# arkworks-rs/accumulation

Hardware: AMD Instinct MI355X
Metric: MSM throughput (point-scalar pairs/sec) at 2^20 Pallas (higher is better)
Workload: dtype u32; 1 GPU; 2^20-pair pallas MSM per GPU (north_star size; scalars uniform in [0, r), G_i = k_i*G), key resident + precomputed window multiples; pairs_per_gpu=1048576, curve=pallas, precomputed_key=True, parallelism=point-sharded x1, window_bits=20, pipeline=bucket-per-lane (k_prep_local_t + k_accum_bpl; skewed scalars re-run chunked), window_widths=9 x 20 + 4 x 19 bits = 256 (MsmGeom::n_narrow), msms_in_flight=3, full=False

## Files before the change

accumulation_amd/csrc/api_entry_ctx.inc:

```

const char* amsm_strerror(int s) {
  switch (s) {
    case AMSM_OK: return "ok";
    case AMSM_E_INVALID_ARG: return "invalid argument";
    case AMSM_E_OOM: return "out of (device) memory";
    case AMSM_E_HIP: return "HIP runtime error";
    case AMSM_E_UNSUPPORTED: return "unsupported size or configuration";
    case AMSM_E_NO_DEVICE: return "no usable gfx950 device (the host backend is never chosen implicitly: ask for AMSM_DEVICE_HOST)";
    case AMSM_E_SCALAR_RANGE: return "scalar out of range (not a canonical into_repr value)";
    case AMSM_E_RCCL: return "RCCL collective failed";
    case AMSM_E_INVALID_POINT: return "invalid point (non-canonical, off the curve or outside the prime-order subgroup)";
    default: return "unknown error";
  }
}

int amsm_device_count(void) {
  int n = 0;
  if (hipGetDeviceCount(&n) != hipSuccess) {
    (void)hipGetLastError();
    return 0;
  }
  return n;
}

// ... 63 lines not shown
    if (hipGetDeviceProperties(&prop, device_id) == hipSuccess && prop.multiProcessorCount > 0) {
      c->cu_count = prop.multiProcessorCount;
      int per_cu = with_curve(curve, [](auto cv) { return accum_l0_blocks_per_cu<typename decltype(cv)::Fq>(); });
      c->wave_slots = prop.multiProcessorCount * std::max(1, per_cu) * 4;
    }
  }
  c->pool_cap_bytes = pool_cap_from_env(c->pool_cap_bytes);
  c->gate.limit = mem_limit_from_env();
  if (const char* e = getenv("AMSM_BPL")) c->bpl = atoi(e) != 0;
  if (const char* e = getenv("AMSM_BPL_PLAIN")) c->bpl_plain = atoi(e) != 0;
  if (const char* e = getenv("AMSM_TOP_SETS")) {
    const int t = atoi(e);
    c->top_sets = (t == 2 || t == 4 || t == 8) ? t : 0;
  }
  if (const char* e = getenv("AMSM_BPL_PROBE")) c->bpl_probe = atoi(e) != 0;
  if (const char* e = getenv("AMSM_BPS")) c->bps = std::max(0, std::min(2, atoi(e)));
  if (const char* e = getenv("AMSM_BPS_BATCH")) c->bps_batch = std::max(0, std::min((int)msel::BPS_BATCH, atoi(e)));
  if (const char* e = getenv("AMSM_SPLIT_LOG2")) c->split_log2 = std::max(0, std::min(28, atoi(e)));
  if (const char* e = getenv("AMSM_DIRECT_SUM_MAX_LOG2")) c->direct_max_log2 = std::max(0, std::min(16, atoi(e)));
  if (const char* e = getenv("AMSM_TWO_VALUED")) c->two_valued = atoi(e) != 0;
  if (const char* e = getenv("AMSM_SHARE_BUCKETS")) c->share_buckets = atoi(e) != 0;
  if (const char* e = getenv("AMSM_HOST_HALVES")) c->host_halves = atoi(e) != 0;
  if (const char* e = getenv("AMSM_SUBGROUP_LADDER")) c->subgroup_ladder = atoi(e) == 2 ? 2 : 1;
  if (const char* e = getenv("AMSM_VEC_SAMPLE_FORM")) c->vec_sample_form = std::max(0, std::min(2, atoi(e)));
  *out = c;
  return AMSM_OK;
}

void amsm_ctx_destroy(amsm_ctx* c) {
  if (!c) return;
// ... 280 lines not shown
```

accumulation_amd/csrc/api_pipeline.inc:

```

#define HIP_TRY(expr)                                                                                  \
  do {                                                                                                 \
    hipError_t _e = (expr);                                                                            \
    if (_e != hipSuccess) {                                                                            \
      fprintf(stderr, "[amsm] HIP error %s (%d) at %s:%d: %s\n", hipGetErrorName(_e), (int)_e, __FILE__, \
              __LINE__, #expr);                                                                        \
      return _e == hipErrorOutOfMemory ? AMSM_E_OOM : AMSM_E_HIP;                                      \
    }                                                                                                  \
  } while (0)

#define TRY(expr)            \
  do {                       \
    int _s = (expr);         \
    if (_s != AMSM_OK) return _s; \
  } while (0)

int ensure(DevBuf& b, size_t bytes) {
  if (b.bytes >= bytes && b.p) return AMSM_OK;
  if (b.p) HIP_TRY(gate_free(b.p));
  b.p = nullptr;
  b.bytes = 0;
  size_t want = bytes + bytes / 8 + 256;
  TRY(gate_alloc(b.owner, GATE_DEVICE, want, false, &b.p));
  b.bytes = want;
// ... 335 lines not shown
  const size_t rec = xyzz_bytes<Fq>();
  if (direct_sum_applies(ctx, job)) {
    DirectPlan dp;
    if (eff) *eff = bases;
    *short_prep_out = false;
    return direct_plan<Fq>(ctx, sl, &job, 1, &dp);
  }
  const msel::Choice ch = choose_pipeline(ctx, bases, n, group_shift, job.force_chunked);
  auto common = [&]() -> int {
    TRY(ensure(sl->buckets, (size_t)g.B * rec));
    return reserve_tail<Fq>(ctx, sl, g.n_sets, msel::tail_plan_any_place(g.nb, g.n_sets, g.B, g.E, g.bpl == 1u));
  };
  if (ch.pipeline == msel::BUCKET_PER_LANE && bpl_geom(ctx, bases, base_off, n, group_shift, ch.plain_window, &g)) {
    sl->geom = g;
    if (eff) *eff = bases;
    TRY(ensure(sl->vals_a, prep_bpl_part_entries(g) * 8 + 64));
    TRY(ensure(sl->vals_b, (size_t)prep_bpl_partitions(g) * prep_bpl_stride(g) * 4 + 64));
    TRY(ensure(sl->bpl_grp, (size_t)prep_bpl_partitions(g) * prep_bpl_groups_per_partition() * 8 + 64));
    TRY(ensure(sl->bpl_order, (size_t)prep_bpl_partitions(g) * prep_bpl_groups_per_partition() * 64 * 4 + 64));
    TRY(common());
    TRY(ensure(sl->prep_small, 64 + prep_small_words(g) * sizeof(u32) + 256));
    *short_prep_out = true;
    return AMSM_OK;
  }
  if (bases->bpl) TRY(bases_alt<Fq>(ctx, bases, &bases));
  if (eff) *eff = bases;
  if (ch.pipeline == msel::BUCKET_SPLIT && bps_geom(ctx, bases, base_off, n, group_shift, &g)) {
    sl->geom = g;
    const u32 P = prep_bps_partitions(g, g.bps_log2_l);
    TRY(ensure(sl->vals_a, prep_bps_part_entries(g, g.bps_log2_l) * 4 + 64));
    TRY(ensure(sl->vals_b, (size_t)P * prep_bps_stride(g, g.bps_log2_l) * 4 + 64));
// ... 107 lines not shown
  u32* d_heavy_count = d_err + 1;
  u32* vals_a = (u32*)sl->vals_a.p;
  u32* vals_b = (u32*)sl->vals_b.p;

  auto prep = [&]() -> int {
    if (!short_prep) HIP_TRY(hipMemsetAsync(sl->misc.p, 0, 64, st));
    stage_mark(ctx, sl, ST_DIGITS, st);
    if (g.bpl) {
      PrepBplBuffers pb;
      pb.d_small = d_err + 16;
      pb.part = vals_a;
      pb.ents_t = vals_b;
      pb.grp = sl->bpl_grp.p;
      pb.order = (u32*)sl->bpl_order.p;
      pb.err = d_err;
      const int rc = g.bpl == 2 ? launch_prep_bps<Fr>(st, (const u32*)d_scalars, scalars_mont, g, g.bps_log2_l, pb)
                                : launch_prep_bpl<Fr>(st, (const u32*)d_scalars, scalars_mont, g, pb);
      if (rc != 0) return AMSM_E_HIP;
      stage_mark(ctx, sl, ST_SORT, st);
      stage_mark(ctx, sl, ST_BOUNDS, st);
      if (g.bpl != 2) ctx->n_bpl++;
      else if (!job.counted) ctx->n_bps++;
      if (g.bpl == 1u && g.top_split) ctx->n_top_sets[(g.top_split + 1u) / 4u]++;
    } else if (short_prep) {
      PrepBuffers pb;
      pb.d_small = d_err + 16;
      pb.part = vals_a;
      pb.vals_sorted = vals_b;
      pb.start = (u32*)sl->start.p;
      pb.items = (u32*)sl->items.p;
// ... 1117 lines not shown
```

accumulation_amd/csrc/api_types.h:

```cpp
#pragma once
struct amsm_ctx;
namespace {

enum Stage { ST_DIGITS = 0, ST_SORT, ST_BOUNDS, ST_ACCUM_L0, ST_ACCUM_L12, ST_REDUCE, ST_COUNT };
const char* kStageNames[ST_COUNT] = {"prep_chain", "prep_sort_rocprim", "prep_bounds_rocprim", "accum_l0", "accum_l1_l2",
                                     "bucket_reduce_fold"};

struct DevBuf {
  void* p = nullptr;
  size_t bytes = 0;
  amsm_ctx* owner = nullptr;
  void release();
};

struct MemGate {
  size_t held = 0, peak = 0;
  size_t limit = 0;
  size_t pinned = 0;
  unsigned long long requests = 0, refused_limit = 0, refused_hook = 0, failed_driver = 0;
  long fail_after = -1;
};

}

// ... 156 lines not shown
  int cu_count = 256;
  unsigned vec_grid_max = 0;
  int wave_slots = 4096;
  bool bpl = true;
  bool bpl_plain = true;
  int top_sets = 0;
  int bps = 2;
  int split_log2 = 21;
  unsigned long long n_bps = 0, n_bps_fallbacks = 0;
  int bps_batch = msel::BPS_BATCH;
  unsigned long long n_bps_units = 0, n_bps_batched = 0, n_bps_unit_reruns = 0;
  unsigned long long n_direct = 0;
  int direct_max_log2 = 15;
  unsigned direct_rr = 0;
  bool host_halves = true;
  bool bpl_probe = true;
  unsigned long long n_top_sets[3] = {0, 0, 0};
  unsigned long long n_bpl = 0, n_bpl_fallbacks = 0;
  bool share_buckets = true;
  DevBuf shared_buckets[2];
  hipEvent_t shared_free[2] = {};
  bool shared_used[2] = {false, false};
  unsigned shared_rr = 0;
  unsigned long long n_shared = 0;
  size_t table_budget = ~(size_t)0;
  unsigned long long n_tables_denied = 0;
  bool profiling = false;
  float stage_ms[ST_COUNT] = {};
  float stage_acc[ST_COUNT] = {};
  int stage_n = 0;
// ... 111 lines not shown
```

accumulation_amd/csrc/kern_fr.hip:

```cpp
#include "launch.h"
#include "vec_kernels.h"
#include "prep_kernels.h"

#include <algorithm>
#include <cmath>
#include <atomic>
#include <cstdlib>
#include <cstring>

namespace amsm {

static inline u32 cdiv_(u32 a, u32 b) { return (a + b - 1) / b; }
void launch_bounds(hipStream_t st, const void* keys_sorted, bool keys16, u32* vals_sorted, MsmGeom g, u32* start,
                   u32* items) {
  if (keys16)
    hipLaunchKernelGGL((k_bounds<uint16_t>), dim3(cdiv_(g.B, 256)), dim3(256), 0, st, (const uint16_t*)keys_sorted,
                       vals_sorted, g, start, items);
  else
    hipLaunchKernelGGL((k_bounds<u32>), dim3(cdiv_(g.B, 256)), dim3(256), 0, st, (const u32*)keys_sorted, vals_sorted,
                       g, start, items);
}

constexpr u32 PREP_MAX_P = 4096;
static PrepGeom prep_geom(const MsmGeom& g) {
// ... 53 lines not shown
  unsigned long long max_idx = (unsigned long long)g.base_off + g.n - 1ull +
                               (g.precomp ? (unsigned long long)(g.W - 1u) * g.table_stride : 0ull);
  if (g.idx_rel_bits) max_idx = ((unsigned long long)(g.W - 1u) << g.idx_rel_bits) | ((1ull << g.idx_rel_bits) - 1ull);
  pg.IB = 1;
  while ((max_idx >> pg.IB) != 0ull) pg.IB++;
  pg.CAP = BPL_LOCAL_BUDGET_WORDS - BPL_LOCAL_FIXED_WORDS;
  pg.HEAVY = 0xffffffffu;
  const unsigned long long per = std::max<unsigned long long>(((unsigned long long)g.E + pg.P - 1) / std::max(1u, pg.P), g.part_max);
  pg.FIX = (u32)std::min<unsigned long long>(pg.CAP, (per + per / 4ull + 2048ull + 15ull) & ~15ull);
  return pg;
}
size_t prep_bpl_part_entries(const MsmGeom& g) {
  PrepGeom pg = prep_bpl_geom(g);
  return std::max<size_t>(g.E, pg.FIX ? (size_t)pg.P * pg.FIX : 0);
}
static size_t prep_bpl_local_lds(const PrepGeom& pg) { return (size_t)(BPL_LOCAL_FIXED_WORDS + pg.CAP) * sizeof(u32); }
static size_t prep_bpl_scatter_lds(const MsmGeom& g, const PrepGeom& pg) {
  const size_t cap = (size_t)pg.SPB * g.S;
  return (3 * (size_t)pg.P + 2 * cap) * sizeof(u32) + cap * sizeof(uint16_t);
}
u32 prep_bpl_partitions(const MsmGeom& g) { return g.B >> 10; }
u32 prep_bpl_groups_per_partition() { return BPL_GROUPS; }
u32 prep_bpl_stride(const MsmGeom& g) {
  const u32 P = std::max(1u, prep_bpl_partitions(g));
  const unsigned long long per = std::max<unsigned long long>(((unsigned long long)g.E + P - 1) / P, g.part_max);
  return (u32)((per + per / 4ull + 4096ull + 1023ull) & ~1023ull);
}
bool prep_bpl_supported(const MsmGeom& g) {
  if (g.S > 32u || g.n == 0 || g.n_sets != g.groups * sets_per_group(g)) return false;
  if (g.B < (1u << 16) || (g.B & 1023u) || (g.B >> 10) > PREP_MAX_P || ((g.B >> 10) & 3u)) return false;
  PrepGeom pg = prep_bpl_geom(g);
  if (pg.IB > 30u) return false;
  if (!msel::bpl_stage_fits(g.E, pg.P, g.part_max, pg.CAP)) return false;
  return prep_bpl_scatter_lds(g, pg) <= PREP_LDS_LIMIT && prep_bpl_local_lds(pg) <= PREP_LDS_LIMIT &&
         (unsigned long long)pg.P * prep_bpl_stride(g) < (1ull << 31);
}
static std::atomic<unsigned long long> prep_bpl_attr_devices{0};
template <class KS>
static void prep_bpl_attr(KS scatter_kernel) {
  int dev = 0;
  if (hipGetDevice(&dev) != hipSuccess || dev < 0 || dev >= 64) dev = 63;
  const unsigned long long bit = 1ull << dev;
  (void)hipFuncSetAttribute((const void*)scatter_kernel, hipFuncAttributeMaxDynamicSharedMemorySize, (int)PREP_LDS_LIMIT);
  if (dev != 63 && (prep_bpl_attr_devices.load(std::memory_order_acquire) & bit)) return;
  static_assert((BPL_LOCAL_BUDGET_WORDS) * sizeof(u32) <= PREP_LDS_LIMIT, "k_prep_local_t's LDS must fit a workgroup");
  (void)hipFuncSetAttribute((const void*)k_prep_local_t, hipFuncAttributeMaxDynamicSharedMemorySize, (int)PREP_LDS_LIMIT);
  prep_bpl_attr_devices.fetch_or(bit, std::memory_order_release);
}

constexpr u32 bps_local_fixed_words(u32 nbp) { return 4u * nbp + 1024u + BPL_BINS + 2u * BPS_GROUPS + 2u; }
constexpr u32 BPS_LOCAL_BUDGET_WORDS = 37888u;
static PrepGeom prep_bps_geom(const MsmGeom& g, u32 log2_l) {
  PrepGeom pg;
  pg.SH = 10u - log2_l;
  pg.P = g.B >> pg.SH;
  pg.SPB = g.S <= 16u ? 512u : 256u;
  unsigned long long max_idx = (unsigned long long)g.base_off + g.n - 1ull +
                               (g.precomp ? (unsigned long long)(g.W - 1u) * g.table_stride : 0ull);
  if (g.idx_rel_bits) max_idx = ((unsigned long long)(g.W - 1u) << g.idx_rel_bits) | ((1ull << g.idx_rel_bits) - 1ull);
  pg.IB = 1;
  while ((max_idx >> pg.IB) != 0ull) pg.IB++;
// ... 208 lines not shown
    PrepGeom pg = prep_bpl_geom(g);                                                                                  \
    u32* part_total = b.d_small;                                                                                     \
    u32* part_start = b.d_small + (PREP_MAX_P + 1);                                                                  \
    u32* part_cursor = b.d_small + 2 * (PREP_MAX_P + 1);                                                             \
    PrepHeavy hv;                                                                                                    \
    hv.n = b.d_small + 4 * (PREP_MAX_P + 1);                                                                         \
    hv.cnt = hv.n + 1;                                                                                               \
    hv.ids = hv.cnt + 64;                                  \
    hv.cur = hv.end = hv.ids;                                                                                        \
    {                  \
      size_t zero_bytes = (16 + 4 * (PREP_MAX_P + 1) + 1) * sizeof(u32);                                             \
      zero_bytes = (zero_bytes + 255) & ~(size_t)255;                                                                \
      if (b.err != b.d_small - 16) return -1;                                                                        \
      if (hipMemsetAsync(b.err, 0, zero_bytes, st) != hipSuccess) return -1;                                         \
    }                                                                                                                \
    if (g.S <= 16u) prep_bpl_attr(k_prep_scatter<FR, 16, 1, true>);                                                  \
    else prep_bpl_attr(k_prep_scatter<FR, 32, 1, true>);                                                             \
    if (!pg.FIX) {                                                                                                   \
      PrepGeom ph = pg;                                                                                              \
      ph.SPB = 1024;                                                                                                 \
      hipLaunchKernelGGL((k_prep_hist<FR>), dim3(cdiv_(g.n, 1024)), dim3(1024), pg.P * sizeof(u32), st, scalars,      \
                         mont, g, ph, part_total, b.err);                                                            \
      hipLaunchKernelGGL(k_prep_scan, dim3(1), dim3(1024), 0, st, part_total, part_start, pg.P, pg.HEAVY, hv);       \
    }                                                                                                                \
    if (g.S <= 16u)                                                                                                  \
      hipLaunchKernelGGL((k_prep_scatter<FR, 16, 1, true>), dim3(cdiv_(g.n, pg.SPB)), dim3(512),                     \
                         prep_bpl_scatter_lds(g, pg), st, scalars, mont, g, pg, part_start, part_cursor, b.part, b.err); \
    else                                             \
      hipLaunchKernelGGL((k_prep_scatter<FR, 32, 1, true>), dim3(cdiv_(g.n, pg.SPB)), dim3(256),                     \
                         prep_bpl_scatter_lds(g, pg), st, scalars, mont, g, pg, part_start, part_cursor, b.part, b.err); \
    hipLaunchKernelGGL(k_prep_local_t, dim3(pg.P), dim3(1024), prep_bpl_local_lds(pg), st,                           \
                       pg.FIX ? part_cursor : part_start, (const u64*)b.part, g, pg, prep_bpl_stride(g), b.ents_t,   \
                       (BplGroup*)b.grp, b.order, b.err);                                                            \
    return 0;                                                                                                        \
  }                                                                                                                  \
  template <>                                                                                                        \
  void launch_digits<FR>(hipStream_t st, const u32* scalars, int mont, MsmGeom g, void* keys, bool keys16, u32* vals, \
                         u32* err) {                                                                                 \
    if (keys16)                                                                                                      \
      hipLaunchKernelGGL((k_digits<FR, uint16_t>), dim3(cdiv_(g.n, 256)), dim3(256), 0, st, scalars, mont, g,         \
                         (uint16_t*)keys, vals, err);                                                                \
    else                                                                                                             \
      hipLaunchKernelGGL((k_digits<FR, u32>), dim3(cdiv_(g.n, 256)), dim3(256), 0, st, scalars, mont, g, (u32*)keys,  \
                         vals, err);                                                                                 \
  }                                                                                                                  \
  template <>                                                                                                        \
  void launch_skew_probe<FR>(hipStream_t st, const u32* scalars, int mont, u32 n, DigitWalk walk, u32* d_flag,       \
                             const u32* d_tv_words) {                                                               \
// ... 125 lines not shown
```

accumulation_amd/csrc/launch.h:

```cpp
#pragma once
#include <hip/hip_runtime.h>

#include <algorithm>

#include "blind.h"
#include "msm_select.h"
#include "msm_types.h"

namespace amsm {

template <class Fq>
void launch_accum_l0(hipStream_t st, const u32* table, const u32* vals_sorted, const u32* start,
                     const u32* item_off, MsmGeom g, u32* partials);
template <class Fq>
void launch_accum_bpl(hipStream_t st, const u32* table, const u32* ents_t, const void* grp, const u32* order, u32 n_groups,
                      u32 groups_per_part, const u32* flags, u32* buckets, u32 wg_per_cu = 0, bool accumulate = false);
template <class Fq>
int accum_l0_blocks_per_cu();
template <class Fq>
void launch_accum_l1(hipStream_t st, u32 lanes_per_bucket, const u32* partials, const u32* items, const u32* item_off, MsmGeom g,
                     u32* buckets, u32* heavy_count, u32* heavy_list);
template <class Fq>
void launch_accum_l2(hipStream_t st, const u32* partials, const u32* items, const u32* item_off,
                     const u32* heavy_count, const u32* heavy_list, u32* scratch, u32* buckets);
// ... 63 lines not shown
  u32* part;
  u32* vals_sorted;
  u32* start;
  u32* items;
  u32* item_off;
  u32* err;
};
bool prep_supported(const MsmGeom& g);
struct PrepBplBuffers {
  u32* d_small;
  u32* part;
  u32* ents_t;
  void* grp;
  u32* order;
  u32* err;
};
bool prep_bpl_supported(const MsmGeom& g);
u32 prep_bpl_stride(const MsmGeom& g);
u32 prep_bpl_partitions(const MsmGeom& g);
size_t prep_bpl_part_entries(const MsmGeom& g);
size_t prep_bps_part_entries(const MsmGeom& g, u32 log2_l);
u32 prep_bpl_groups_per_partition();
template <class Fr>
int launch_prep_bpl(hipStream_t st, const u32* scalars, int mont, MsmGeom g, const PrepBplBuffers& b);
int prep_bps_choose(const MsmGeom& g);
u32 prep_bps_partitions(const MsmGeom& g, u32 log2_l);
u32 prep_bps_stride(const MsmGeom& g, u32 log2_l);
template <class Fr>
int launch_prep_bps(hipStream_t st, const u32* scalars, int mont, MsmGeom g, u32 log2_l, const PrepBplBuffers& b);
template <class Fq>
void launch_accum_bps(hipStream_t st, const u32* table, const u32* ents_t, const void* grp, const u32* order, u32 n_groups,
                      u32 log2_l, const u32* flags, u32* buckets);
struct BpsBatchBuffers {
  u32* small;
  u32 small_stride;
// ... 76 lines not shown
```

accumulation_amd/csrc/msm_select.h:

```cpp
#pragma once
#include <math.h>
#include <stddef.h>

#include <initializer_list>

namespace amsm {
namespace msel {

enum Pipeline { DIRECT_SUM = 0, BUCKET_SPLIT = 1, BUCKET_PER_LANE = 2, CHUNKED = 3 };
inline const char* pipeline_name(int p) {
  return p == DIRECT_SUM ? "direct_sum" : (p == BUCKET_SPLIT ? "bucket_split" : (p == BUCKET_PER_LANE ? "bucket_per_lane" : "chunked"));
}

inline int ilog2_ceil(size_t n) {
  int l = 0;
  while (((size_t)1 << l) < n) l++;
  return l;
}
constexpr size_t P2(int k) { return (size_t)1 << k; }

constexpr int BPL_WINDOW = 20;
constexpr int DIRECT_MAX_LOG2 = 15;
struct KeyWindowRow {
  int lg_lo, lg_hi;
// ... 194 lines not shown
      const char *a0 = vec[v].scalars, *a1 = a0 + vec[v].n * 32;
      for (size_t u = 0; u < k && verdict[v] == V_ONES_APART; u++) {
        if (u == v || verdict[u] != V_REGULAR || vec[u].n == 0) continue;
        const char *b0 = vec[u].scalars, *b1 = b0 + vec[u].n * 32;
        if (a0 < b1 && b0 < a1) verdict[v] = V_REGULAR, changed = true;
      }
    }
  }
}

constexpr unsigned BPL_STAGE_CAP = 37340;
inline bool bpl_stage_fits(unsigned long long E, unsigned long long P, unsigned long long part_max, unsigned cap) {
  if (P == 0 || E / P + 1024ull > cap) return false;
  return !(part_max && part_max + 5ull * (unsigned long long)sqrt((double)part_max) > cap);
}
inline unsigned long long plain_part_max(size_t n, unsigned nb, unsigned long long reach, unsigned T, unsigned groups) {
  const unsigned long long per_win = ((unsigned long long)n * 1024ull + nb - 1) / nb;
  const unsigned long long per_top = ((unsigned long long)n * 1024ull + reach - 1) / reach;
  const unsigned long long top = (2ull * per_top + T - 1) / T;
  const unsigned long long pm = per_win > top ? per_win : top;
  return groups > 1u ? (pm + 1ull) / 2ull : pm;
}
inline unsigned plain_top_sets(size_t n, unsigned nb, unsigned long long reach, unsigned W, unsigned groups, unsigned cap = BPL_STAGE_CAP,
                               unsigned max_sets = 8) {
  if (n == 0 || nb < 1024u || reach == 0 || W == 0) return 0;
  for (unsigned T = 2; T <= max_sets && T <= 8u; T *= 2u) {
    const unsigned long long P = ((unsigned long long)groups * (W + T) * nb) >> 10;
    if (bpl_stage_fits((unsigned long long)n * W, P, plain_part_max(n, nb, reach, T, groups), cap)) return T;
  }
  return 0;
// ... 82 lines not shown
```

accumulation_amd/csrc/prep_kernels.h:

```cpp
#pragma once
#include "fp.h"
#include "msm_select.h"
#include "msm_types.h"
#include "vec_kernels.h"

namespace amsm {

struct PrepGeom {
  u32 SH;
  u32 P;
  u32 SPB;
  u32 IB;
  u32 CAP;
  u32 HEAVY;
  u32 FIX;
};

constexpr u32 PREP_HEAVY_SLICES = 64, PREP_HEAVY_GRID = 1024, PREP_MAX_HEAVY = 4096;
struct PrepHeavy {
  u32* n;
  u32* ids;
  u32* cnt;
  u32* cur;
  u32* end;
};

constexpr u32 PREP_ENTRY_LAST = 0x40000000u;

AMSM_DEV u32 lds_count(u32* ctr, u32 idx) {
  const u64 active = __ballot(1);
// ... 91 lines not shown
    u32 v = in[k];
    out[k] = run;
    run += v;
  }
  if (with_total && t == T - 1) out[n] = lds[T - 1];
}

__global__ void __launch_bounds__(1024)
    k_prep_scan(const u32* __restrict__ part_total, u32* __restrict__ part_start, u32 P, u32 heavy_min, PrepHeavy hv) {
  __shared__ u32 lds[1024];
  block_exclusive_scan(part_total, part_start, P, true, lds);
  for (u32 p = threadIdx.x; p < P; p += blockDim.x)
    if (part_total[p] > heavy_min) hv.ids[atomicAdd(hv.n, 1u)] = p;
}

template <class Fr, int MAXW, int SPT, bool WIDE>
AMSM_DEV void prep_scatter_body(const u32* scalars, int mont, MsmGeom g, PrepGeom pg, const u32* part_start, u32* part_cursor, u32* part,
                                u32* err) {
  extern __shared__ u32 prep_lds[];
  const u32 cap = pg.SPB * g.S;
  u32* cnt = prep_lds;
  u32* loff = prep_lds + pg.P;
  u32* gbase = prep_lds + 2 * pg.P;
  u32* staged = prep_lds + 3 * pg.P;
  uint16_t* staged_p = reinterpret_cast<uint16_t*>(staged + (WIDE ? 2u : 1u) * cap);
  const u32 t = threadIdx.x, T = blockDim.x;
  for (u32 p = t; p < pg.P; p += T) cnt[p] = 0;
  __syncthreads();
  u32 rk[SPT][MAXW / 2];
  Fe<Fr> sreg[SPT];
#pragma unroll
  for (int r = 0; r < SPT; r++) {
#pragma unroll
// ... 3 lines not shown
      sreg[r] = fe_load<Fr>(scalars + (size_t)i * 8);
      if (g.skip_ones) fe_drop_stored_one<Fr>(sreg[r], mont);
      if (mont) sreg[r] = fe_from_mont<Fr>(sreg[r]);
      const u32 bad = scalar_entries_unrolled_reg<Fr, MAXW>(sreg[r], g, i, [&](int w, u32 key, u32) {
        u32 rank = atomicAdd(&cnt[key >> pg.SH], 1u);
        rk[r][w >> 1] |= rank << ((w & 1) * 16);
      });
      if (pg.FIX && bad && err) atomicOr(err, 1u);
    }
  }
  __syncthreads();
  constexpr u32 RSV_MAX = 4;
  u32 rsv[RSV_MAX], rsv_base[RSV_MAX];
  u32 per = (pg.P + T - 1) / T;
  u32 lo = min(t * per, pg.P), hi = min(lo + per, pg.P);
  {
    u32* sl = reinterpret_cast<u32*>(staged);
    u32 sum = 0;
    for (u32 p = lo; p < hi; p++) sum += cnt[p];
    sl[t] = sum;
    __syncthreads();
    for (u32 d = 1; d < T; d <<= 1) {
      u32 v = t >= d ? sl[t - d] : 0u;
      __syncthreads();
      sl[t] += v;
      __syncthreads();
    }
    u32 run = sl[t] - sum;
#pragma unroll
    for (u32 q = 0; q < RSV_MAX; q++) {
      u32 p = lo + q;
      rsv[q] = 0;
      rsv_base[q] = 0;
      if (p < hi) {
        u32 v = cnt[p];
        loff[p] = run;
        if (v) {
          rsv_base[q] = pg.FIX ? p * pg.FIX : part_start[p];
          rsv[q] = atomicAdd(&part_cursor[p], v);
        }
        run += v;
      }
    }
    for (u32 p = lo + RSV_MAX; p < hi; p++) {
      u32 v = cnt[p];
      loff[p] = run;
      gbase[p] = v ? (pg.FIX ? p * pg.FIX : part_start[p]) + atomicAdd(&part_cursor[p], v) : 0u;
      run += v;
    }
  }
  __syncthreads();
  const u32 low = (1u << pg.SH) - 1u;
#pragma unroll
  for (int r = 0; r < SPT; r++) {
    u32 i = blockIdx.x * pg.SPB + r * T + t;
    if (i < g.n)
      scalar_entries_unrolled_reg<Fr, MAXW>(sreg[r], g, i, [&](int w, u32 key, u32 val) {
        u32 p = key >> pg.SH;
        u32 rank = (rk[r][w >> 1] >> ((w & 1) * 16)) & 0xffffu;
        u32 slot = loff[p] + rank;
        if (WIDE) reinterpret_cast<u64*>(staged)[slot] = ((u64)(key & low) << 32) | val;
        else staged[slot] = (val & 0x80000000u) | ((key & low) << pg.IB) | (val & 0x7fffffffu);
        staged_p[slot] = (uint16_t)p;
      });
  }
#pragma unroll
  for (u32 q = 0; q < RSV_MAX; q++)
    if (lo + q < hi) gbase[lo + q] = rsv_base[q] + rsv[q];
  __syncthreads();
  u32 total = loff[pg.P - 1] + cnt[pg.P - 1];
  for (u32 j = t; j < total; j += T) {
    u32 p = staged_p[j];
    const u32 dst = gbase[p] + (j - loff[p]);
    if (pg.FIX && dst - p * pg.FIX >= pg.FIX) continue;
    if (WIDE) reinterpret_cast<u64*>(part)[dst] = reinterpret_cast<const u64*>(staged)[j];
    else part[dst] = staged[j];
  }
}
template <class Fr, int MAXW, int SPT, bool WIDE = false>
__global__ void __launch_bounds__(512)
    k_prep_scatter(const u32* __restrict__ scalars, int mont, MsmGeom g, PrepGeom pg, const u32* __restrict__ part_start,
                   u32* __restrict__ part_cursor, u32* __restrict__ part, u32* __restrict__ err = nullptr) {
  prep_scatter_body<Fr, MAXW, SPT, WIDE>(scalars, mont, g, pg, part_start, part_cursor, part, err);
}
constexpr int PREP_BPS_BATCH = msel::BPS_BATCH;
struct BpsBatchScalars {
  const u32* scalars[PREP_BPS_BATCH];
};
template <class Fr, int MAXW, int SPT>
__global__ void __launch_bounds__(512)
    k_prep_scatter_batch(BpsBatchScalars b, int mont, MsmGeom g, PrepGeom pg, const u32* __restrict__ part_start0,
                         u32* __restrict__ part_cursor0, u32 small_stride, u32* __restrict__ part0, u32 part_stride,
                         u32* __restrict__ err) {
  const size_t v = blockIdx.y;
  prep_scatter_body<Fr, MAXW, SPT, false>(b.scalars[v], mont, g, pg, part_start0 + v * small_stride, part_cursor0 + v * small_stride,
                                          part0 + v * part_stride, err);
}

// ... 250 lines not shown
  __syncthreads();
  u32 before = 0;
#pragma unroll
  for (u32 i = 0; i < 15u; i++) before += i < w ? wt[i] : 0u;
  return v + before;
}

constexpr u32 BPL_LOCAL_SLOTS = 37, BPL_SLOT_BLOCK = 8;
template <class F>
AMSM_DEV void bpl_slot_blocks(u32 n, F&& f) {
#pragma unroll
  for (u32 b = 0; b < BPL_LOCAL_SLOTS; b += BPL_SLOT_BLOCK)
    if (b * BPL_NB < n) f(b);
}

__global__ void __launch_bounds__(1024)
    k_prep_local_t(const u32* __restrict__ part_start, const u64* __restrict__ part, MsmGeom g, PrepGeom pg, u32 stride,
                   u32* __restrict__ ents_t, BplGroup* __restrict__ grp, u32* __restrict__ order, u32* __restrict__ err) {
  extern __shared__ u32 prep_lds[];
  constexpr u32 NB = BPL_NB, NG = BPL_GROUPS, T = BPL_NB, SLOTS = BPL_LOCAL_SLOTS, BLK = BPL_SLOT_BLOCK;
  u32* cnt = prep_lds;
  u32* cur = cnt + NB;
  u32* wt = cur + NB;
  u32* bins = wt + NB;
  u32* first = bins + BPL_BINS;
  u32* gm = first + BPL_BINS;
  u32* stage = gm + 2u * NG + 1u;
  const u32 p = blockIdx.x, t = threadIdx.x;
  const u32 ps = pg.FIX ? p * pg.FIX : part_start[p];
  const u32 n_p = pg.FIX ? part_start[p] : part_start[p + 1] - ps;
  const u32 pe = ps + (pg.FIX ? min(n_p, pg.FIX) : n_p);
  const u32 low = NB - 1u, idx_mask = (1u << pg.IB) - 1u, b0 = p << pg.SH;
  const bool fits = n_p <= pg.CAP && (!pg.FIX || n_p <= pg.FIX);
  const u32 n = fits ? min(pe - ps, SLOTS * T) : 0u;
  u64 e[SLOTS];
#pragma unroll
  for (u32 i = 0; i < SLOTS; i++) e[i] = 0;
  bpl_slot_blocks(n, [&](u32 b) {
#pragma unroll
    for (u32 i = b; i < b + BLK && i < SLOTS; i++) e[i] = part[ps + min(i * T + t, n - 1u)];
  });
  cnt[t] = 0;
  if (t < BPL_BINS) bins[t] = 0;
  if (t < NG) gm[t] = 0;
  __syncthreads();
  bpl_slot_blocks(n, [&](u32 b) {
#pragma unroll
    for (u32 i = b; i < b + BLK && i < SLOTS; i++)
      if (i * T + t < n) atomicAdd(&cnt[(u32)(e[i] >> 32) & low], 1u);
  });
  __syncthreads();
  const u32 c_t = cnt[t];
  const u32 first_t = block_scan_inclusive(c_t, wt) - c_t;
  cur[t] = first_t;
  const u32 bin = min(c_t, BPL_BINS - 1u);
  const u32 rank = atomicAdd(&bins[bin], 1u);
  __syncthreads();
  bpl_slot_blocks(n, [&](u32 b) {
    u32 pos[BLK];
#pragma unroll
    for (u32 i = b; i < b + BLK && i < SLOTS; i++) {
      pos[i - b] = 0;
      if (i * T + t < n) pos[i - b] = atomicAdd(&cur[(u32)(e[i] >> 32) & low], 1u);
    }
#pragma unroll
    for (u32 i = b; i < b + BLK && i < SLOTS; i++) {
      const u32 lo = (u32)e[i];
      if (i * T + t < n) stage[pos[i - b]] = (lo & 0x80000000u) | entry_abs_index(g, lo & idx_mask);
    }
  });
  const u32 in_class = t < BPL_BINS ? bins[BPL_BINS - 1u - t] : 0u;
  const u32 larger = block_scan_inclusive(in_class, wt + 16) - in_class;
  if (t < BPL_BINS) first[BPL_BINS - 1u - t] = larger;
  __syncthreads();
  const u32 my_pos = first[bin] + rank;
  cnt[my_pos] = c_t;
  cur[my_pos] = first_t;
  {
    const u32 h0 = (c_t + 1u) >> 1;
    if (my_pos < BPL_SPLIT / 2u) atomicMax(&gm[0], h0);
    else if (my_pos < BPL_SPLIT) atomicMax(&gm[NG - 1u], h0);
    else atomicMax(&gm[my_pos / BPL_GROUP], c_t);
  }
  __syncthreads();
  u32 total = 0, my_gb = 0;
// ... 161 lines not shown
```

Baseline: 986.5 million pairs/s.

## Pack bucket-per-lane prep entries into one 32-bit word with sub-range cursors

Adds a narrow entry form for the bucket-per-lane prep. Each partition entry becomes one u32 holding the sign, local bucket and window, plus a point offset relative to a sub-range. Points are split into G sub-ranges with their own cursors and capacities. The aim is to halve the global traffic and the scatter LDS between k_prep_scatter and k_prep_local_t. The cost is extra geometry logic and more capacity-overflow conditions, and the wide u64 form is kept behind AMSM_BPL_WIDE as a fallback.

```diff
diff --git a/accumulation_amd/csrc/api_entry_ctx.inc b/accumulation_amd/csrc/api_entry_ctx.inc
--- a/accumulation_amd/csrc/api_entry_ctx.inc
+++ b/accumulation_amd/csrc/api_entry_ctx.inc
@@ -101,6 +101,7 @@
     c->top_sets = (t == 2 || t == 4 || t == 8) ? t : 0;
   }
   if (const char* e = getenv("AMSM_BPL_PROBE")) c->bpl_probe = atoi(e) != 0;
+  if (const char* e = getenv("AMSM_BPL_WIDE")) c->bpl_wide = atoi(e) != 0;
   if (const char* e = getenv("AMSM_BPS")) c->bps = std::max(0, std::min(2, atoi(e)));
   if (const char* e = getenv("AMSM_BPS_BATCH")) c->bps_batch = std::max(0, std::min((int)msel::BPS_BATCH, atoi(e)));
   if (const char* e = getenv("AMSM_SPLIT_LOG2")) c->split_log2 = std::max(0, std::min(28, atoi(e)));
diff --git a/accumulation_amd/csrc/api_pipeline.inc b/accumulation_amd/csrc/api_pipeline.inc
--- a/accumulation_amd/csrc/api_pipeline.inc
+++ b/accumulation_amd/csrc/api_pipeline.inc
@@ -373,7 +373,7 @@
   if (ch.pipeline == msel::BUCKET_PER_LANE && bpl_geom(ctx, bases, base_off, n, group_shift, ch.plain_window, &g)) {
     sl->geom = g;
     if (eff) *eff = bases;
-    TRY(ensure(sl->vals_a, prep_bpl_part_entries(g) * 8 + 64));
+    TRY(ensure(sl->vals_a, prep_bpl_part_entries(g) * prep_bpl_entry_bytes(g, ctx->bpl_wide) + 64));
     TRY(ensure(sl->vals_b, (size_t)prep_bpl_partitions(g) * prep_bpl_stride(g) * 4 + 64));
     TRY(ensure(sl->bpl_grp, (size_t)prep_bpl_partitions(g) * prep_bpl_groups_per_partition() * 8 + 64));
     TRY(ensure(sl->bpl_order, (size_t)prep_bpl_partitions(g) * prep_bpl_groups_per_partition() * 64 * 4 + 64));
@@ -511,6 +511,7 @@
       pb.grp = sl->bpl_grp.p;
       pb.order = (u32*)sl->bpl_order.p;
       pb.err = d_err;
+      pb.wide = ctx->bpl_wide;
       const int rc = g.bpl == 2 ? launch_prep_bps<Fr>(st, (const u32*)d_scalars, scalars_mont, g, g.bps_log2_l, pb)
                                 : launch_prep_bpl<Fr>(st, (const u32*)d_scalars, scalars_mont, g, pb);
       if (rc != 0) return AMSM_E_HIP;
diff --git a/accumulation_amd/csrc/api_types.h b/accumulation_amd/csrc/api_types.h
--- a/accumulation_amd/csrc/api_types.h
+++ b/accumulation_amd/csrc/api_types.h
@@ -194,6 +194,7 @@
   int direct_max_log2 = 15;
   unsigned direct_rr = 0;
   bool host_halves = true;
+  bool bpl_wide = false;
   bool bpl_probe = true;
   unsigned long long n_top_sets[3] = {0, 0, 0};
   unsigned long long n_bpl = 0, n_bpl_fallbacks = 0;
diff --git a/accumulation_amd/csrc/kern_fr.hip b/accumulation_amd/csrc/kern_fr.hip
--- a/accumulation_amd/csrc/kern_fr.hip
+++ b/accumulation_amd/csrc/kern_fr.hip
@@ -91,10 +91,24 @@
   PrepGeom pg = prep_bpl_geom(g);
   return std::max<size_t>(g.E, pg.FIX ? (size_t)pg.P * pg.FIX : 0);
 }
+static_assert(msel::BPL_SUB_BUCKET_BITS == 10 && BPL_NB == (1u << msel::BPL_SUB_BUCKET_BITS), "a partition is 2^10 buckets");
+static_assert(msel::BPL_SUB_MAX * msel::BPL_SUB_SLOTS * BPL_NB >= BPL_LOCAL_BUDGET_WORDS - BPL_LOCAL_FIXED_WORDS,
+              "k_prep_local_t<false>'s register slots hold a whole stage");
+static_assert(msel::BPL_SUB_MAX * msel::BPL_SUB_SLOTS <= 2u * BPL_LOCAL_SLOTS, "one-word slots take no more registers than the wide ones");
+static_assert(msel::BPL_SUB_FIX_CONST == 2048u, "prep_bpl_geom: the constant of FIX");
+constexpr u32 BPL_CURSOR_WORDS = 2u * (PREP_MAX_P + 1u);
+static msel::BplEntryForm prep_bpl_form(const MsmGeom& g, const PrepGeom& pg, bool wide) {
+  const unsigned long long per = std::max<unsigned long long>(((unsigned long long)g.E + pg.P - 1) / std::max(1u, pg.P), g.part_max);
+  const msel::BplEntryForm f = msel::bpl_entry_form(g.n, g.W, g.precomp != 0u, pg.P, per, pg.FIX, BPL_CURSOR_WORDS, wide);
+  if (f.narrow && f.G > 1u && g.groups > 1u && g.group_shift >= f.lbits)
+    return msel::bpl_entry_form(g.n, g.W, g.precomp != 0u, pg.P, per, pg.FIX, BPL_CURSOR_WORDS, true);
+  return f;
+}
+size_t prep_bpl_entry_bytes(const MsmGeom& g, bool wide) { return prep_bpl_form(g, prep_bpl_geom(g), wide).narrow ? 4 : 8; }
 static size_t prep_bpl_local_lds(const PrepGeom& pg) { return (size_t)(BPL_LOCAL_FIXED_WORDS + pg.CAP) * sizeof(u32); }
-static size_t prep_bpl_scatter_lds(const MsmGeom& g, const PrepGeom& pg) {
+static size_t prep_bpl_scatter_lds(const MsmGeom& g, const PrepGeom& pg, bool narrow = false) {
   const size_t cap = (size_t)pg.SPB * g.S;
-  return (3 * (size_t)pg.P + 2 * cap) * sizeof(u32) + cap * sizeof(uint16_t);
+  return (3 * (size_t)pg.P + (narrow ? 1 : 2) * cap) * sizeof(u32) + cap * sizeof(uint16_t);
 }
 u32 prep_bpl_partitions(const MsmGeom& g) { return g.B >> 10; }
 u32 prep_bpl_groups_per_partition() { return BPL_GROUPS; }
@@ -121,7 +135,8 @@
   (void)hipFuncSetAttribute((const void*)scatter_kernel, hipFuncAttributeMaxDynamicSharedMemorySize, (int)PREP_LDS_LIMIT);
   if (dev != 63 && (prep_bpl_attr_devices.load(std::memory_order_acquire) & bit)) return;
   static_assert((BPL_LOCAL_BUDGET_WORDS) * sizeof(u32) <= PREP_LDS_LIMIT, "k_prep_local_t's LDS must fit a workgroup");
-  (void)hipFuncSetAttribute((const void*)k_prep_local_t, hipFuncAttributeMaxDynamicSharedMemorySize, (int)PREP_LDS_LIMIT);
+  (void)hipFuncSetAttribute((const void*)k_prep_local_t<true>, hipFuncAttributeMaxDynamicSharedMemorySize, (int)PREP_LDS_LIMIT);
+  (void)hipFuncSetAttribute((const void*)k_prep_local_t<false>, hipFuncAttributeMaxDynamicSharedMemorySize, (int)PREP_LDS_LIMIT);
   prep_bpl_attr_devices.fetch_or(bit, std::memory_order_release);
 }
 
@@ -360,6 +375,28 @@
       if (b.err != b.d_small - 16) return -1;                                                                        \
       if (hipMemsetAsync(b.err, 0, zero_bytes, st) != hipSuccess) return -1;                                         \
     }                                                                                                                \
+    const msel::BplEntryForm form = prep_bpl_form(g, pg, b.wide);                                                    \
+    if (form.narrow) {           \
+      PrepSub sub;                                                                                                   \
+      sub.G = form.G;                                                                                                \
+      sub.lbits = form.lbits;                                                                                        \
+      sub.wmask = (1u << form.wbits) - 1u;                                                                           \
+      sub.stride = form.cap_full;                                                                                    \
+      sub.cap_full = form.cap_full;                                                                                  \
+      sub.cap_last = form.cap_last;                                                                                  \
+      if (g.S <= 16u) {                                                                                              \
+        prep_bpl_attr(k_prep_scatter_sub<FR, 16, 1>);                                                                \
+        hipLaunchKernelGGL((k_prep_scatter_sub<FR, 16, 1>), dim3(cdiv_(g.n, pg.SPB)), dim3(512),                     \
+                           prep_bpl_scatter_lds(g, pg, true), st, scalars, mont, g, pg, sub, part_cursor, b.part, b.err); \
+      } else {                                                                                                       \
+        prep_bpl_attr(k_prep_scatter_sub<FR, 32, 1>);                                                                \
+        hipLaunchKernelGGL((k_prep_scatter_sub<FR, 32, 1>), dim3(cdiv_(g.n, pg.SPB)), dim3(256),                     \
+                           prep_bpl_scatter_lds(g, pg, true), st, scalars, mont, g, pg, sub, part_cursor, b.part, b.err); \
+      }                                                                                                              \
+      hipLaunchKernelGGL(k_prep_local_t<false>, dim3(pg.P), dim3(1024), prep_bpl_local_lds(pg), st, part_cursor,     \
+                         (const void*)b.part, g, pg, sub, prep_bpl_stride(g), b.ents_t, (BplGroup*)b.grp, b.order, b.err); \
+      return 0;                                                                                                      \
+    }                                                                                                                \
     if (g.S <= 16u) prep_bpl_attr(k_prep_scatter<FR, 16, 1, true>);                                                  \
     else prep_bpl_attr(k_prep_scatter<FR, 32, 1, true>);                                                             \
     if (!pg.FIX) {                                                                                                   \
@@ -375,9 +412,9 @@
     else                                             \
       hipLaunchKernelGGL((k_prep_scatter<FR, 32, 1, true>), dim3(cdiv_(g.n, pg.SPB)), dim3(256),                     \
                          prep_bpl_scatter_lds(g, pg), st, scalars, mont, g, pg, part_start, part_cursor, b.part, b.err); \
-    hipLaunchKernelGGL(k_prep_local_t, dim3(pg.P), dim3(1024), prep_bpl_local_lds(pg), st,                           \
-                       pg.FIX ? part_cursor : part_start, (const u64*)b.part, g, pg, prep_bpl_stride(g), b.ents_t,   \
-                       (BplGroup*)b.grp, b.order, b.err);                                                            \
+    hipLaunchKernelGGL(k_prep_local_t<true>, dim3(pg.P), dim3(1024), prep_bpl_local_lds(pg), st,                     \
+                       pg.FIX ? part_cursor : part_start, (const void*)b.part, g, pg, PrepSub{}, prep_bpl_stride(g), \
+                       b.ents_t, (BplGroup*)b.grp, b.order, b.err);                                                  \
     return 0;                                                                                                        \
   }                                                                                                                  \
   template <>                                                                                                        \
diff --git a/accumulation_amd/csrc/launch.h b/accumulation_amd/csrc/launch.h
--- a/accumulation_amd/csrc/launch.h
+++ b/accumulation_amd/csrc/launch.h
@@ -101,11 +101,13 @@
   void* grp;
   u32* order;
   u32* err;
+  bool wide = false;
 };
 bool prep_bpl_supported(const MsmGeom& g);
 u32 prep_bpl_stride(const MsmGeom& g);
 u32 prep_bpl_partitions(const MsmGeom& g);
 size_t prep_bpl_part_entries(const MsmGeom& g);
+size_t prep_bpl_entry_bytes(const MsmGeom& g, bool wide);
 size_t prep_bps_part_entries(const MsmGeom& g, u32 log2_l);
 u32 prep_bpl_groups_per_partition();
 template <class Fr>
diff --git a/accumulation_amd/csrc/msm_select.h b/accumulation_amd/csrc/msm_select.h
--- a/accumulation_amd/csrc/msm_select.h
+++ b/accumulation_amd/csrc/msm_select.h
@@ -232,6 +232,51 @@
   if (P == 0 || E / P + 1024ull > cap) return false;
   return !(part_max && part_max + 5ull * (unsigned long long)sqrt((double)part_max) > cap);
 }
+constexpr unsigned BPL_SUB_MAX = 8, BPL_SUB_SLOTS = 5, BPL_SUB_BUCKET_BITS = 10, BPL_SUB_FIX_CONST = 2048;
+struct BplEntryForm {
+  unsigned narrow;
+  unsigned wbits;
+  unsigned lbits;
+  unsigned G;
+  unsigned cap_full;
+  unsigned cap_last;
+  unsigned slots;
+};
+inline BplEntryForm bpl_entry_form(unsigned long long n, unsigned W, bool precomp, unsigned long long P, unsigned long long per,
+                                   unsigned fix, unsigned long long cursor_words, bool force_wide) {
+  BplEntryForm f{};
+  f.G = 1;
+  f.cap_full = f.cap_last = fix;
+  if (force_wide || fix == 0 || n == 0 || P == 0) return f;
+  unsigned wbits = 0;
+  if (precomp)
+    while (((W - 1u) >> wbits) != 0u) wbits++;
+  const unsigned room = 31u - BPL_SUB_BUCKET_BITS;
+  if (wbits + 9u > room) return f;
+  const unsigned lbits = room - wbits;
+  const unsigned long long full = 1ull << lbits, G = (n + full - 1ull) / full;
+  if (G > BPL_SUB_MAX || P * G > cursor_words) return f;
+  if (G == 1ull) {
+    if (fix > BPL_SUB_MAX * BPL_SUB_SLOTS * 1024u) return f;
+    f.slots = (fix + 1023u) / 1024u;
+  } else {
+    const unsigned long long last = n - (G - 1ull) * full;
+    const unsigned long long b_full = per * full / n, b_last = per * last / n, k = BPL_SUB_FIX_CONST / G;
+    f.cap_full = (unsigned)((b_full + b_full / 4ull + k) & ~15ull);
+    f.cap_last = (unsigned)((b_last + b_last / 4ull + k) & ~15ull);
+    if (f.cap_full > BPL_SUB_SLOTS * 1024u || (G - 1ull) * f.cap_full + f.cap_last > fix) {
+      f.cap_full = f.cap_last = fix;
+      return f;
+    }
+    f.slots = (unsigned)(G - 1ull) * ((f.cap_full + 1023u) / 1024u) + (f.cap_last + 1023u) / 1024u;
+  }
+  f.narrow = 1;
+  f.wbits = wbits;
+  f.lbits = lbits;
+  f.G = (unsigned)G;
+  return f;
+}
+
 inline unsigned long long plain_part_max(size_t n, unsigned nb, unsigned long long reach, unsigned T, unsigned groups) {
   const unsigned long long per_win = ((unsigned long long)n * 1024ull + nb - 1) / nb;
   const unsigned long long per_top = ((unsigned long long)n * 1024ull + reach - 1) / reach;
diff --git a/accumulation_amd/csrc/prep_kernels.h b/accumulation_amd/csrc/prep_kernels.h
--- a/accumulation_amd/csrc/prep_kernels.h
+++ b/accumulation_amd/csrc/prep_kernels.h
@@ -14,6 +14,15 @@
   u32 CAP;
   u32 HEAVY;
   u32 FIX;
+};
+
+constexpr u32 BPL_SUB_IDX_BITS = 31u - msel::BPL_SUB_BUCKET_BITS;
+struct PrepSub {
+  u32 G;
+  u32 lbits;
+  u32 wmask;
+  u32 stride;
+  u32 cap_full, cap_last;
 };
 
 constexpr u32 PREP_HEAVY_SLICES = 64, PREP_HEAVY_GRID = 1024, PREP_MAX_HEAVY = 4096;
@@ -135,9 +144,10 @@
     if (part_total[p] > heavy_min) hv.ids[atomicAdd(hv.n, 1u)] = p;
 }
 
-template <class Fr, int MAXW, int SPT, bool WIDE>
+template <class Fr, int MAXW, int SPT, bool WIDE, bool SUB = false>
 AMSM_DEV void prep_scatter_body(const u32* scalars, int mont, MsmGeom g, PrepGeom pg, const u32* part_start, u32* part_cursor, u32* part,
-                                u32* err) {
+                                u32* err, const PrepSub sub = PrepSub{}) {
+  static_assert(!(WIDE && SUB), "one-word entries are the alternative to the wide form");
   extern __shared__ u32 prep_lds[];
   const u32 cap = pg.SPB * g.S;
   u32* cnt = prep_lds;
@@ -171,6 +181,11 @@
   u32 rsv[RSV_MAX], rsv_base[RSV_MAX];
   u32 per = (pg.P + T - 1) / T;
   u32 lo = min(t * per, pg.P), hi = min(lo + per, pg.P);
+  const u32 sub_r = SUB ? (blockIdx.x * pg.SPB) >> sub.lbits : 0u;
+  const u32 sub_off = SUB ? sub_r * sub.stride : 0u;
+  const u32 sub_cap = SUB ? (sub_r + 1u == sub.G ? sub.cap_last : sub.cap_full) : pg.FIX;
+  auto run_base = [&](u32 p) { return SUB ? p * pg.FIX + sub_off : (pg.FIX ? p * pg.FIX : part_start[p]); };
+  auto cursor_of = [&](u32 p) { return SUB ? p * sub.G + sub_r : p; };
   {
     u32* sl = reinterpret_cast<u32*>(staged);
     u32 sum = 0;
@@ -193,8 +208,8 @@
         u32 v = cnt[p];
         loff[p] = run;
         if (v) {
-          rsv_base[q] = pg.FIX ? p * pg.FIX : part_start[p];
-          rsv[q] = atomicAdd(&part_cursor[p], v);
+          rsv_base[q] = run_base(p);
+          rsv[q] = atomicAdd(&part_cursor[cursor_of(p)], v);
         }
         run += v;
       }
@@ -202,7 +217,7 @@
     for (u32 p = lo + RSV_MAX; p < hi; p++) {
       u32 v = cnt[p];
       loff[p] = run;
-      gbase[p] = v ? (pg.FIX ? p * pg.FIX : part_start[p]) + atomicAdd(&part_cursor[p], v) : 0u;
+      gbase[p] = v ? run_base(p) + atomicAdd(&part_cursor[cursor_of(p)], v) : 0u;
       run += v;
     }
   }
@@ -217,6 +232,9 @@
         u32 rank = (rk[r][w >> 1] >> ((w & 1) * 16)) & 0xffffu;
         u32 slot = loff[p] + rank;
         if (WIDE) reinterpret_cast<u64*>(staged)[slot] = ((u64)(key & low) << 32) | val;
+        else if (SUB)
+          staged[slot] = (val & 0x80000000u) | ((key & low) << BPL_SUB_IDX_BITS) | (((u32)w & sub.wmask) << sub.lbits) |
+                         (i & ((1u << sub.lbits) - 1u));
         else staged[slot] = (val & 0x80000000u) | ((key & low) << pg.IB) | (val & 0x7fffffffu);
         staged_p[slot] = (uint16_t)p;
       });
@@ -229,7 +247,9 @@
   for (u32 j = t; j < total; j += T) {
     u32 p = staged_p[j];
     const u32 dst = gbase[p] + (j - loff[p]);
-    if (pg.FIX && dst - p * pg.FIX >= pg.FIX) continue;
+    if (SUB) {
+      if (dst - (p * pg.FIX + sub_off) >= sub_cap) continue;
+    } else if (pg.FIX && dst - p * pg.FIX >= pg.FIX) continue;
     if (WIDE) reinterpret_cast<u64*>(part)[dst] = reinterpret_cast<const u64*>(staged)[j];
     else part[dst] = staged[j];
   }
@@ -239,6 +259,12 @@
     k_prep_scatter(const u32* __restrict__ scalars, int mont, MsmGeom g, PrepGeom pg, const u32* __restrict__ part_start,
                    u32* __restrict__ part_cursor, u32* __restrict__ part, u32* __restrict__ err = nullptr) {
   prep_scatter_body<Fr, MAXW, SPT, WIDE>(scalars, mont, g, pg, part_start, part_cursor, part, err);
+}
+template <class Fr, int MAXW, int SPT>
+__global__ void __launch_bounds__(512)
+    k_prep_scatter_sub(const u32* __restrict__ scalars, int mont, MsmGeom g, PrepGeom pg, PrepSub sub, u32* __restrict__ part_cursor,
+                       u32* __restrict__ part, u32* __restrict__ err) {
+  prep_scatter_body<Fr, MAXW, SPT, false, true>(scalars, mont, g, pg, nullptr, part_cursor, part, err, sub);
 }
 constexpr int PREP_BPS_BATCH = msel::BPS_BATCH;
 struct BpsBatchScalars {
@@ -519,8 +545,9 @@
     if (b * BPL_NB < n) f(b);
 }
 
+template <bool WIDE>
 __global__ void __launch_bounds__(1024)
-    k_prep_local_t(const u32* __restrict__ part_start, const u64* __restrict__ part, MsmGeom g, PrepGeom pg, u32 stride,
+    k_prep_local_t(const u32* __restrict__ part_start, const void* __restrict__ part_v, MsmGeom g, PrepGeom pg, PrepSub sub, u32 stride,
                    u32* __restrict__ ents_t, BplGroup* __restrict__ grp, u32* __restrict__ order, u32* __restrict__ err) {
   extern __shared__ u32 prep_lds[];
   constexpr u32 NB = BPL_NB, NG = BPL_GROUPS, T = BPL_NB, SLOTS = BPL_LOCAL_SLOTS, BLK = BPL_SLOT_BLOCK;
@@ -532,48 +559,121 @@
   u32* gm = first + BPL_BINS;
   u32* stage = gm + 2u * NG + 1u;
   const u32 p = blockIdx.x, t = threadIdx.x;
-  const u32 ps = pg.FIX ? p * pg.FIX : part_start[p];
-  const u32 n_p = pg.FIX ? part_start[p] : part_start[p + 1] - ps;
-  const u32 pe = ps + (pg.FIX ? min(n_p, pg.FIX) : n_p);
-  const u32 low = NB - 1u, idx_mask = (1u << pg.IB) - 1u, b0 = p << pg.SH;
-  const bool fits = n_p <= pg.CAP && (!pg.FIX || n_p <= pg.FIX);
-  const u32 n = fits ? min(pe - ps, SLOTS * T) : 0u;
-  u64 e[SLOTS];
-#pragma unroll
-  for (u32 i = 0; i < SLOTS; i++) e[i] = 0;
-  bpl_slot_blocks(n, [&](u32 b) {
-#pragma unroll
-    for (u32 i = b; i < b + BLK && i < SLOTS; i++) e[i] = part[ps + min(i * T + t, n - 1u)];
-  });
-  cnt[t] = 0;
-  if (t < BPL_BINS) bins[t] = 0;
-  if (t < NG) gm[t] = 0;
-  __syncthreads();
-  bpl_slot_blocks(n, [&](u32 b) {
-#pragma unroll
-    for (u32 i = b; i < b + BLK && i < SLOTS; i++)
-      if (i * T + t < n) atomicAdd(&cnt[(u32)(e[i] >> 32) & low], 1u);
-  });
-  __syncthreads();
-  const u32 c_t = cnt[t];
-  const u32 first_t = block_scan_inclusive(c_t, wt) - c_t;
-  cur[t] = first_t;
-  const u32 bin = min(c_t, BPL_BINS - 1u);
-  const u32 rank = atomicAdd(&bins[bin], 1u);
-  __syncthreads();
-  bpl_slot_blocks(n, [&](u32 b) {
-    u32 pos[BLK];
-#pragma unroll
-    for (u32 i = b; i < b + BLK && i < SLOTS; i++) {
-      pos[i - b] = 0;
-      if (i * T + t < n) pos[i - b] = atomicAdd(&cur[(u32)(e[i] >> 32) & low], 1u);
-    }
-#pragma unroll
-    for (u32 i = b; i < b + BLK && i < SLOTS; i++) {
-      const u32 lo = (u32)e[i];
-      if (i * T + t < n) stage[pos[i - b]] = (lo & 0x80000000u) | entry_abs_index(g, lo & idx_mask);
-    }
-  });
+  const u32 low = NB - 1u, b0 = p << pg.SH;
+  bool fits;
+  u32 c_t, first_t, bin, rank;
+  if constexpr (WIDE) {
+    const u64* __restrict__ part = static_cast<const u64*>(part_v);
+    const u32 ps = pg.FIX ? p * pg.FIX : part_start[p];
+    const u32 n_p = pg.FIX ? part_start[p] : part_start[p + 1] - ps;
+    const u32 pe = ps + (pg.FIX ? min(n_p, pg.FIX) : n_p);
+    const u32 idx_mask = (1u << pg.IB) - 1u;
+    fits = n_p <= pg.CAP && (!pg.FIX || n_p <= pg.FIX);
+    const u32 n = fits ? min(pe - ps, SLOTS * T) : 0u;
+    u64 e[SLOTS];
+#pragma unroll
+    for (u32 i = 0; i < SLOTS; i++) e[i] = 0;
+    bpl_slot_blocks(n, [&](u32 b) {
+#pragma unroll
+      for (u32 i = b; i < b + BLK && i < SLOTS; i++) e[i] = part[ps + min(i * T + t, n - 1u)];
+    });
+    cnt[t] = 0;
+    if (t < BPL_BINS) bins[t] = 0;
+    if (t < NG) gm[t] = 0;
+    __syncthreads();
+    bpl_slot_blocks(n, [&](u32 b) {
+#pragma unroll
+      for (u32 i = b; i < b + BLK && i < SLOTS; i++)
+        if (i * T + t < n) atomicAdd(&cnt[(u32)(e[i] >> 32) & low], 1u);
+    });
+    __syncthreads();
+    c_t = cnt[t];
+    first_t = block_scan_inclusive(c_t, wt) - c_t;
+    cur[t] = first_t;
+    bin = min(c_t, BPL_BINS - 1u);
+    rank = atomicAdd(&bins[bin], 1u);
+    __syncthreads();
+    bpl_slot_blocks(n, [&](u32 b) {
+      u32 pos[BLK];
+#pragma unroll
+      for (u32 i = b; i < b + BLK && i < SLOTS; i++) {
+        pos[i - b] = 0;
+        if (i * T + t < n) pos[i - b] = atomicAdd(&cur[(u32)(e[i] >> 32) & low], 1u);
+      }
+#pragma unroll
+      for (u32 i = b; i < b + BLK && i < SLOTS; i++) {
+        const u32 lo = (u32)e[i];
+        if (i * T + t < n) stage[pos[i - b]] = (lo & 0x80000000u) | entry_abs_index(g, lo & idx_mask);
+      }
+    });
+  } else {
+    constexpr u32 NR = msel::BPL_SUB_MAX, SPR = msel::BPL_SUB_SLOTS;
+    const u32* __restrict__ part = static_cast<const u32*>(part_v);
+    const u32 ps = p * pg.FIX;
+    u32 nr[NR], n = 0;
+    fits = true;
+#pragma unroll
+    for (u32 r = 0; r < NR; r++) {
+      if (sub.G > 1u) {
+        const u32 c = r < sub.G ? part_start[p * sub.G + r] : 0u, cap = r + 1u == sub.G ? sub.cap_last : sub.cap_full;
+        fits = fits && c <= cap;
+        nr[r] = min(c, cap);
+      } else {
+        const u32 c = part_start[p], m = min(c, pg.FIX);
+        fits = fits && c <= pg.FIX;
+        nr[r] = min(m - min(m, r * SPR * T), SPR * T);
+      }
+      n += nr[r];
+    }
+    fits = fits && n <= pg.CAP;
+    const u32 sub_stride = sub.G > 1u ? sub.stride : SPR * T;
+    u32 e[NR * SPR];
+#pragma unroll
+    for (u32 r = 0; r < NR; r++) {
+      const u32 n_r = fits ? nr[r] : 0u;
+#pragma unroll
+      for (u32 k = 0; k < SPR; k++) {
+        e[r * SPR + k] = 0;
+        if (k * T < n_r) e[r * SPR + k] = part[ps + r * sub_stride + min(k * T + t, n_r - 1u)];
+      }
+    }
+    cnt[t] = 0;
+    if (t < BPL_BINS) bins[t] = 0;
+    if (t < NG) gm[t] = 0;
+    __syncthreads();
+#pragma unroll
+    for (u32 r = 0; r < NR; r++) {
+      const u32 n_r = fits ? nr[r] : 0u;
+#pragma unroll
+      for (u32 k = 0; k < SPR; k++)
+        if (k * T + t < n_r) atomicAdd(&cnt[(e[r * SPR + k] >> BPL_SUB_IDX_BITS) & low], 1u);
+    }
+    __syncthreads();
+    c_t = cnt[t];
+    first_t = block_scan_inclusive(c_t, wt) - c_t;
+    cur[t] = first_t;
+    bin = min(c_t, BPL_BINS - 1u);
+    rank = atomicAdd(&bins[bin], 1u);
+    __syncthreads();
+    const u32 lmask = (1u << sub.lbits) - 1u;
+#pragma unroll
+    for (u32 r = 0; r < NR; r++) {
+      const u32 n_r = fits ? nr[r] : 0u;
+      const u32 idx_r = g.base_off + (sub.G > 1u ? r << sub.lbits : 0u);
+      u32 pos[SPR];
+#pragma unroll
+      for (u32 k = 0; k < SPR; k++) {
+        pos[k] = 0;
+        if (k * T + t < n_r) pos[k] = atomicAdd(&cur[(e[r * SPR + k] >> BPL_SUB_IDX_BITS) & low], 1u);
+      }
+#pragma unroll
+      for (u32 k = 0; k < SPR; k++) {
+        const u32 v = e[r * SPR + k];
+        if (k * T + t < n_r)
+          stage[pos[k]] = (v & 0x80000000u) | (idx_r + (v & lmask) + ((v >> sub.lbits) & sub.wmask) * g.table_stride);
+      }
+    }
+  }
   const u32 in_class = t < BPL_BINS ? bins[BPL_BINS - 1u - t] : 0u;
   const u32 larger = block_scan_inclusive(in_class, wt + 16) - in_class;
   if (t < BPL_BINS) first[BPL_BINS - 1u - t] = larger;
```

After: 994.4 million pairs/s, median of 6. No clear change (+0.8%).
